# kamperh/segmentalist

Measured on AMD Instinct MI355X. Metric: Gibbs sweeps/sec (10k utts, D=100, K=1000) at 1/2/4/8 MI355X, higher is better.
Workload: dtype fp16 one-product filter + fp16x2 second stage, float32 reference arithmetic for the results; 1 GPU; SegmentalKMeansWordseg batch-synchronous sweep (BASELINE.json configs[2]); utterances=10000, landmarks_per_utt=20, n_slices_max=6, embeddings=1050000, D=100, K=1000, parallelism=utterance shards x1, ONE all-gather of the packed block statistics per sweep, collective=none (single process), sweep_launch=plain launches, corpus=one device holds all rows, device_memory_allocated_bytes_rank0=1237140992, components_after=815

## Files before the change

### include/segk.h

```cpp
#ifndef SEGK_H
#define SEGK_H

#include <stdint.h>

#ifdef __cplusplus
extern "C" {
#endif

#define SEGK_OK 0
#define SEGK_ERR_ARG (-1)
#define SEGK_ERR_HIP (-2)
#define SEGK_ERR_NO_DEVICE (-3)
#define SEGK_ERR_UNSUPPORTED (-4)

#define SEGK_F32 0
#define SEGK_F64 1

typedef struct segk_ctx segk_ctx;

int32_t segk_create(int32_t device_id, segk_ctx **out_ctx);
int32_t segk_destroy(segk_ctx *ctx);
const char *segk_last_error(void);
#define SEGK_ABI_VERSION 15
int32_t segk_abi_version(void);
// ... 103 lines not shown

int32_t segk_kmeans_update_utt(segk_ctx *ctx, const segk_corpus *c, segk_kmeans *m,
                               int32_t utt, const int32_t *old_tok, const int32_t *new_tok,
                               const int32_t *new_k, const int32_t *n_old, const int32_t *n_new,
                               int32_t *status, void *stream);

int32_t segk_kmeans_add_item(segk_ctx *ctx, const segk_corpus *c, segk_kmeans *m, int64_t i,
                             int32_t k, int32_t *status, void *stream);
int32_t segk_kmeans_del_item(segk_ctx *ctx, const segk_corpus *c, segk_kmeans *m, int64_t i,
                             int32_t *status, void *stream);
int32_t segk_kmeans_clean_components(segk_ctx *ctx, const segk_corpus *c, segk_kmeans *m,
                                     int32_t *status, void *stream);

int32_t segk_kmeans_del_component(segk_ctx *ctx, const segk_corpus *c, segk_kmeans *m, int32_t k,
                                  int32_t *status, void *stream);

int32_t segk_kmeans_sequential_sweep(segk_ctx *ctx, const segk_corpus *c, segk_kmeans *m,
                                     const int32_t *order, int32_t n_order, int32_t n_slices_min,
                                     int32_t n_slices_max, double wip, const segk_cand *cand,
                                     uint64_t *keys_scratch, uint8_t *boundaries, int32_t *old_tok,
                                     int32_t *new_tok, int32_t *new_k, int32_t *n_old, int32_t *n_new,
                                     int32_t *n_flag, double *out_total, int32_t *status, void *stream);

int64_t segk_kmeans_batch_record_words(int32_t K_max, int32_t D, int32_t n_blocks_local, int32_t flag_cap,
                                       int32_t flag_row_bytes);
int32_t segk_kmeans_batch_scratch_words(int32_t K_max, int64_t n_slots, int32_t n_blocks_local, int64_t *sorted_words,
                                        int64_t *koff_words);
int32_t segk_kmeans_batch_partials(segk_ctx *ctx, const segk_corpus *c, const segk_kmeans *m,
                                   const int32_t *blk_lo, int32_t n_blocks_local,
                                   const int32_t *new_tok, const int32_t *new_k, const int32_t *n_flag,
                                   const double *out_total, int32_t *sorted_scratch,
                                   int32_t *koff_scratch, double *record, int32_t flag_cap, int32_t flag_rows,
                                   double *out_scalars, void *stream);
int32_t segk_kmeans_batch_finalize(segk_ctx *ctx, const segk_corpus *c, segk_kmeans *m,
                                   int32_t utt_lo, int32_t utt_hi, const double *records,
                                   int32_t n_blocks_total, int32_t n_blocks_per_rank,
                                   int64_t rank_stride, int32_t flag_cap, int32_t flag_rows, int32_t my_rank,
                                   int32_t *new_k, int32_t *remap_scratch, double *out_scalars,
                                   int32_t *status, void *stream);
int32_t segk_kmeans_batch_record(segk_ctx *ctx, const segk_corpus *c, const segk_kmeans *m, int32_t utt_lo,
                                 int32_t utt_hi, const int32_t *new_tok, const int32_t *new_k,
                                 const int32_t *status, double *out_scalars, void *stream);
int32_t segk_kmeans_assignments_from_tokens(segk_ctx *ctx, const segk_corpus *c, segk_kmeans *m,
                                            int32_t utt_lo, int32_t utt_hi, const int32_t *new_tok,
                                            const int32_t *new_k, const int32_t *n_new,
                                            void *stream);

int64_t segk_kmeans_refit_scratch_words(int64_t n_slots);
int32_t segk_kmeans_refit_collect(segk_ctx *ctx, const segk_corpus *c, int32_t utt_lo, int32_t utt_hi,
                                  const int32_t *new_tok, const int32_t *new_k, int32_t *chunk_scratch,
                                  int32_t *ids, int32_t *slots, int64_t n_list, int32_t *count_out,
                                  int32_t *status, void *stream);
int32_t segk_kmeans_refit_apply(segk_ctx *ctx, const segk_corpus *c, const segk_kmeans *m,
                                const segk_cand *cand, int32_t utt_lo, int32_t utt_hi,
                                const int32_t *new_tok, int32_t *new_k, int32_t *n_flag, int32_t *moved,
                                int32_t *status, void *stream);
int32_t segk_kmeans_hint_relabel(segk_ctx *ctx, const segk_corpus *c, const segk_kmeans *m,
                                 const segk_cand *cand, const int32_t *table, void *stream);
int32_t segk_kmeans_refit_record(segk_ctx *ctx, const segk_corpus *c, const segk_kmeans *m, int32_t utt_lo,
                                 int32_t utt_hi, const int32_t *new_tok, const int32_t *new_k,
                                 const int32_t *status, const int32_t *moved, double *out_scalars,
                                 void *stream);

int64_t segk_kmeans_fit_scratch_words(int64_t n_emb, int64_t n_items_max, int32_t K_max);
int32_t segk_kmeans_fit_step(segk_ctx *ctx, const segk_corpus *c, segk_kmeans *m, const segk_cand *cand,
                             int32_t consider_unassigned, int64_t n_items_max, int32_t *scratch, double *record,
// ... 193 lines not shown
```

### segmentalist_amd/_abi.py

```python
import ctypes as C
import os
import subprocess

_HERE = os.path.dirname(os.path.abspath(__file__))
LIB_PATH = os.environ.get("SEGK_LIB_PATH") or os.path.join(_HERE, "libsegk.so")

SEGK_F32, SEGK_F64 = 0, 1
SEGK_ERR_UNSUPPORTED = -4
ABI_VERSION = 15


class SegkError(RuntimeError):
    pass


class Corpus(C.Structure):
    _fields_ = [
        ("X", C.c_void_p), ("X32", C.c_void_p), ("x_dtype", C.c_int32), ("D", C.c_int32),
        ("n_emb", C.c_int64), ("ldx", C.c_int64), ("ld32", C.c_int64), ("xnorm", C.c_void_p),
        ("vec_ids", C.c_void_p), ("durations", C.c_void_p), ("lengths", C.c_void_p),
        ("n_utt", C.c_int32), ("N_max", C.c_int32), ("Xb3", C.c_void_p), ("sp_pieces", C.c_int32), ("band_W", C.c_int32),
        ("band_ids", C.c_void_p), ("band_dur", C.c_void_p),
    ]

# ... 43 lines not shown
    "segk_create": (_i32, [_i32, C.POINTER(_P)]),
    "segk_destroy": (_i32, [_P]),
    "segk_last_error": (C.c_char_p, []),
    "segk_abi_version": (_i32, []),
    "segk_corpus_prepare": (_i32, [_P, _CP, _P, _P, _P]),
    "segk_kmeans_tiles_floats": (_i64, [_i32, _i32]),
    "segk_kmeans_prepare": (_i32, [_P, _CP, _KP, _P]),
    "segk_kmeans_mark_duplicates": (_i32, [_P, _CP, _KP, _P, _P]),
    "segk_kmeans_init_stats": (_i32, [_P, _CP, _KP, _P]),
    "segk_kmeans_score": (_i32, [_P, _CP, _KP, _P, _i64, _i64, _DP, _P, _P]),
    "segk_kmeans_score_hinted": (_i32, [_P, _CP, _KP, _P, _i64, _i64, _DP, _P, _P, _P]),
    "segk_kmeans_clear_queue": (_i32, [_P, _DP, _P]),
    "segk_kmeans_filter": (_i32, [_P, _CP, _KP, _P, _i64, _i64, _DP, _P]),
    "segk_kmeans_resolve": (_i32, [_P, _CP, _KP, _P, _i64, _i64, _DP, _P, _P]),
    "segk_kmeans_stage_counts": (_i32, [_P, _DP, C.POINTER(_i32), _P]),
    "segk_kmeans_hint_feedback": (_i32, [_P, C.POINTER(C.c_uint32), C.POINTER(C.c_uint32), C.POINTER(_i32)]),
    "segk_kmeans_delta_stats": (_i32, [_P, C.POINTER(_i32)]),
    "segk_kmeans_exact_max": (_i32, [_P, _CP, _KP, _P, _i64, _DP, _P, _P, _P]),
    "segk_kmeans_neg_sqrd_norm": (_i32, [_P, _CP, _KP, _i64, _P, _P]),
    "segk_kmeans_segment": (_i32, [_P, _CP, _KP, _P, _i32, _i32, _i32, _i32, _f64, _DP, _P, _P, _P, _P, _P, _P,
                                   _P, _P, _P, _P]),
    "segk_dp_tri": (_i32, [_P, _i32, _P, _P, _P, _i32, _i32, _i32, _f64, _f64, _P, _i64, _P, _i64, _P, _P, _P,
                           _P, _i64, _P]),
    "segk_kmeans_update_utt": (_i32, [_P, _CP, _KP, _i32, _P, _P, _P, _P, _P, _P, _P]),
    "segk_kmeans_sequential_sweep": (_i32, [_P, _CP, _KP, _P, _i32, _i32, _i32, _f64, _DP, _P, _P, _P, _P, _P, _P, _P, _P, _P,
                                            _P, _P]),
    "segk_kmeans_add_item": (_i32, [_P, _CP, _KP, _i64, _i32, _P, _P]),
    "segk_kmeans_del_item": (_i32, [_P, _CP, _KP, _i64, _P, _P]),
    "segk_kmeans_clean_components": (_i32, [_P, _CP, _KP, _P, _P]),
    "segk_kmeans_del_component": (_i32, [_P, _CP, _KP, _i32, _P, _P]),
    "segk_kmeans_batch_record_words": (_i64, [_i32, _i32, _i32, _i32, _i32]),
    "segk_kmeans_batch_scratch_words": (_i32, [_i32, _i64, _i32, C.POINTER(_i64), C.POINTER(_i64)]),
    "segk_kmeans_batch_partials": (_i32, [_P, _CP, _KP, _P, _i32, _P, _P, _P, _P, _P, _P, _P, _i32, _i32, _P, _P]),
    "segk_kmeans_batch_finalize": (_i32, [_P, _CP, _KP, _i32, _i32, _P, _i32, _i32, _i64, _i32, _i32, _i32, _P, _P, _P, _P,
                                          _P]),
    "segk_kmeans_batch_record": (_i32, [_P, _CP, _KP, _i32, _i32, _P, _P, _P, _P, _P]),
    "segk_kmeans_assignments_from_tokens": (_i32, [_P, _CP, _KP, _i32, _i32, _P, _P, _P, _P]),
    "segk_kmeans_refit_scratch_words": (_i64, [_i64]),
    "segk_kmeans_refit_collect": (_i32, [_P, _CP, _i32, _i32, _P, _P, _P, _P, _P, _i64, _P, _P, _P]),
    "segk_kmeans_refit_apply": (_i32, [_P, _CP, _KP, _DP, _i32, _i32, _P, _P, _P, _P, _P, _P]),
    "segk_kmeans_hint_relabel": (_i32, [_P, _CP, _KP, _DP, _P, _P]),
    "segk_kmeans_refit_record": (_i32, [_P, _CP, _KP, _i32, _i32, _P, _P, _P, _P, _P, _P]),
    "segk_kmeans_fit_scratch_words": (_i64, [_i64, _i64, _i32]),
    "segk_kmeans_fit_step": (_i32, [_P, _CP, _KP, _DP, _i32, _i64, _P, _P, _P, _P]),
    "segk_kmeans_sum_neg_sqrd_norm": (_i32, [_P, _CP, _KP, _P, _P]),
    "segk_fbgmm_record_metrics": (_i32, [_P, _CP, _FP, _i32, _f64, _P, _P]),
    "segk_fbgmm_init_stats": (_i32, [_P, _CP, _FP, _P]),
    "segk_fbgmm_update": (_i32, [_P, _CP, _FP, _i32, _i32, _i64, _i32, _P, _P]),
    "segk_fbgmm_score": (_i32, [_P, _CP, _FP, _P, _i64, _i64, _P, _P]),
    "segk_fbgmm_pred_vector": (_i32, [_P, _CP, _FP, _i64, _P, _P]),
    "segk_unigram_segment": (_i32, [_P, _CP, _i32, _i32, _i32, _i32, _f64, _f64, _f64, _f64, _P, _P, _P, _i64, _P,
                                    _P, _P, _P, _P, _P]),
    "segk_fbgmm_assign": (_i32, [_P, _CP, _FP, _i32, _i32, _i32, _f64, _P, _P, _P, _P, _i64, _P, _P]),
    "segk_fbgmm_gibbs_items": (_i32, [_P, _CP, _FP, _P, _i64, _i32, _f64, _P, _P, _i64, _P, _P]),
    "segk_fbgmm_sequential_sweep": (_i32, [_P, _CP, _FP, _P, _i32, _P, _i32, _i32, _i32, _i32, _f64, _f64, _f64, _f64, _f64,
                                           _P, _P, _P, _i64, _P, _P, _P, _P, _P, _P]),
    "segk_fbb_collect": (_i32, [_P, _CP, _P, _P, _P, _P]),
    "segk_fbb_partials": (_i32, [_P, _CP, _FP, _BP, _i32, _i32, _i32, _P, _P, _P]),
    "segk_fbb_prepare": (_i32, [_P, _CP, _FP, _BP, _i32, _P]),
    "segk_fbb_score": (_i32, [_P, _CP, _FP, _BP, _i32, _i32, _i32, _P, _P, _P]),
    "segk_fbb_score_diag32": (_i32, [_P, _CP, _FP, _BP, _i32, _i32, _i32, _P, _P, _P]),
    "segk_calibrate_vlog": (_i32, [_P, C.POINTER(_f64), _P]),
    "segk_fbb_make_y": (_i32, [_P, _CP, _BP, _P]),
    "segk_fbb_prior_rows": (_i32, [_P, _CP, _FP, _P, _P]),
    "segk_fbb_score_f32": (_i32, [_P, _CP, _FP, _BP, _P, _i64, _P, _P]),
    "segk_fbb_segment": (_i32, [_P, _CP, _FP, _BP, _i32, _i32, _i32, _P, _u64, _i32, _i32, _f64, _f64, _f64, _P, _P,
# ... 103 lines not shown
```

### segmentalist_amd/csrc/segk_stats.hip

```cpp
#include "segk_kmeans_dev.h"


template <typename XT>
__device__ void dev_del_component(const segk_corpus &c, segk_kmeans &m, int k, int *shK, int32_t *relog = nullptr)
{
    const int tid = threadIdx.x, nt = blockDim.x;
    const int D = c.D;
    const int K = *shK;
    XT *means = (XT *)m.means;
    const XT *rnd = (const XT *)m.random_means;
    if (k != K) {
        const double cntK = (double)m.counts[K];
        for (int d = tid; d < D; d += nt) {
            double v = m.mean_numerators[(int64_t)K * D + d];
            m.mean_numerators[(int64_t)k * D + d] = v;
            means[(int64_t)k * D + d] = (XT)(v / cntK);
        }
        if (relog) {
            if (tid == 0) {
                const int n = relog[0];
                relog[1 + 2 * n] = K;
                relog[2 + 2 * n] = k;
                relog[0] = n + 1;
            }
// ... 523 lines not shown
    double s = 0.0;
    for (int uc = u0; uc < u1; uc += 2048) {
        const int nu = u1 - uc < 2048 ? u1 - uc : 2048;
        __syncthreads();
        for (int i = tid; i < nu; i += SORT_THREADS) stage[i] = out_total[uc + i];
        __syncthreads();
        if (tid == 0) {
            int i = 0;
            for (; i + 16 <= nu; i += 16) {
                double v[16];
#pragma unroll
                for (int q = 0; q < 16; q++) v[q] = stage[i + q];
#pragma unroll
                for (int q = 0; q < 16; q++) s += v[q];
            }
            for (; i < nu; i++) s += stage[i];
        }
    }
    if (tid == 0) part_tot[b] = s;
    SEGK_TSTAMP(1, 4);
}

#define SORT_CL 512
static inline __host__ __device__ int segk_sort_rsh(int K_max) { return K_max <= 2048 ? 5 : 7; }
static inline __host__ __device__ int segk_sort_nsh(int K_max)
{
    const int need = (K_max + (1 << segk_sort_rsh(K_max)) - 1) >> segk_sort_rsh(K_max);
    int nsh = 0;
    while ((1 << nsh) < need) nsh++;
    return nsh;
}
static inline __host__ __device__ int segk_sort_ranges(int K_max) { return 1 << segk_sort_nsh(K_max); }

__global__ __launch_bounds__(SORT_THREADS) void k_batch_sort_sum(
    segk_corpus c, segk_kmeans m, const int32_t *blk_lo, int n_blocks, const int32_t *new_tok, const int32_t *new_k,
    const double *out_total, int32_t *sorted, int32_t *koff2, double *part_tot, int32_t *flags, int cap, double *out_scalars, int NR,
    int rsh, int nsh, double *part_sum, int64_t *part_cnt, int fuse_sum)
{
    extern __shared__ __attribute__((aligned(16))) unsigned char sort_lds[];
    __shared__ int32_t wcount[16], wscan[2];
    const int tid = threadIdx.x, lane = tid & 63, wv = tid >> 6;
    const int Kb = *m.K;
    const int K_max = m.K_max;
    const int RS = 1 << rsh, kmask = RS - 1;
    const int b = blockIdx.x / (NR + 2), r = blockIdx.x % (NR + 2);
    const int u0 = blk_lo[b], u1 = blk_lo[b + 1];
    SEGK_TSTAMP(1, 0);
    if (r == NR + 1) {
        if (b == 0 && tid == 0) {
            *(double *)m.mnorm_max = 0.0;
            out_scalars[3] = (double)Kb;
        }
        double *stage = reinterpret_cast<double *>(sort_lds);
        double s = 0.0;
        for (int uc = u0; uc < u1; uc += 2048) {
            const int nu = u1 - uc < 2048 ? u1 - uc : 2048;
            __syncthreads();
            for (int i = tid; i < nu; i += SORT_THREADS) stage[i] = out_total[uc + i];
            __syncthreads();
            if (tid == 0) {
                int i = 0;
                for (; i + 16 <= nu; i += 16) {
                    double v[16];
#pragma unroll
                    for (int q = 0; q < 16; q++) v[q] = stage[i + q];
#pragma unroll
                    for (int q = 0; q < 16; q++) s += v[q];
                }
                for (; i < nu; i++) s += stage[i];
            }
        }
        if (tid == 0) part_tot[b] = s;
        SEGK_TSTAMP(1, 4);
        return;
    }
    const bool flg = r == NR;
    const int64_t p0 = (int64_t)u0 * c.N_max;
    const int S = (u1 - u0) * c.N_max;
    const int per = ((S + 15) / 16 + 63) & ~63;
    const bool preload = per <= 2048;
    int32_t *cntw = reinterpret_cast<int32_t *>(sort_lds);
    int32_t *base = cntw + 16 * RS;
    int32_t *cnts = base + RS;
    uint32_t *cl = reinterpret_cast<uint32_t *>(cnts + RS) + (size_t)wv * SORT_CL;
    const int32_t *keys = new_k + (S > 0 ? p0 : 0);
    const int s0 = wv * per < S ? wv * per : S, s1 = s0 + per < S ? s0 + per : S;
    auto in_range = [&](int k) -> bool { return flg ? k >= Kb : (k >= 0 && k < Kb && (k & (NR - 1)) == r); };
    for (int i = tid; i < 16 * RS; i += SORT_THREADS) cntw[i] = 0;
    int n_mine = 0;
    if (preload) {
        constexpr int NC = 2048 / 64;
        int v[NC];
#pragma unroll
        for (int q = 0; q < NC; q++) {
            const int sidx = s0 + q * 64 + lane;
            v[q] = keys[sidx < s1 ? sidx : (S > 0 ? S - 1 : 0)];
        }
        __syncthreads();
#pragma unroll
        for (int q = 0; q < NC; q++) {
            if (s0 + q * 64 >= s1) break;
            const int sidx = s0 + q * 64 + lane;
            const int k = sidx < s1 ? v[q] : -1;
            const bool in = sidx < s1 && in_range(k);
            const unsigned long long bal = __ballot(in);
            if (in) {
                const int at = n_mine + __popcll(bal & ((1ull << lane) - 1ull));
                if (at < SORT_CL) cl[at] = ((unsigned int)sidx << rsh) | (unsigned int)((k >> nsh) & kmask);
                if (!flg) atomicAdd(&cntw[wv * RS + ((k >> nsh) & kmask)], 1);
            }
            n_mine += __popcll(bal);
        }
    } else {
        __syncthreads();
        for (int sb = s0; sb < s1; sb += 64) {
            const int sidx = sb + lane;
            const int k = sidx < s1 ? keys[sidx] : -1;
            const bool in = sidx < s1 && in_range(k);
            if (in && !flg) atomicAdd(&cntw[wv * RS + ((k >> nsh) & kmask)], 1);
            n_mine += __popcll(__ballot(in));
        }
    }
    if (lane == 0) wcount[wv] = n_mine;
    const bool compact = !__syncthreads_or(!preload || n_mine > SORT_CL);
    SEGK_TSTAMP(1, 2);
    if (flg) {
        int32_t *fl = flags + (int64_t)b * 2 * segk_flag_words(cap);
        int off = 0, tot = 0;
        for (int w = 0; w < 16; w++) {
            if (w < wv) off += wcount[w];
            tot += wcount[w];
        }
        if (tid == 0) { fl[0] = tot; fl[1] = 0; }
        if (compact) {
            for (int i = lane; i < n_mine; i += 64) {
                const int sidx = (int)(cl[i] >> rsh);
                if (off + i < cap) {
                    fl[2 + 3 * (off + i) + 0] = (int32_t)(p0 + sidx);
                    fl[2 + 3 * (off + i) + 1] = keys[sidx];
                    fl[2 + 3 * (off + i) + 2] = new_tok[p0 + sidx];
                }
            }
        } else {
            int done = 0;
            for (int sb = s0; sb < s1 && done < n_mine; sb += 64) {
                const int sidx = sb + lane;
                const int k = sidx < s1 ? keys[sidx] : -1;
                const bool in = sidx < s1 && k >= Kb;
                const unsigned long long bal = __ballot(in);
                const int at = off + done + __popcll(bal & ((1ull << lane) - 1ull));
                if (in && at < cap) {
                    fl[2 + 3 * at + 0] = (int32_t)(p0 + sidx);
                    fl[2 + 3 * at + 1] = k;
                    fl[2 + 3 * at + 2] = new_tok[p0 + sidx];
                }
                done += __popcll(bal);
            }
        }
        SEGK_TSTAMP_MAX(1, 4);
        return;
    }
    int run = 0, incl = 0;
    if (tid < RS) {
        int t[16];
#pragma unroll
        for (int w = 0; w < 16; w++) t[w] = cntw[w * RS + tid];
#pragma unroll
        for (int w = 0; w < 16; w++) {
            cntw[w * RS + tid] = run;
            run += t[w];
        }
        incl = run;
        for (int o = 1; o < 64; o <<= 1) {
            const int t2 = __shfl_up(incl, o);
            if (lane >= o) incl += t2;
        }
        if (lane == 63) wscan[wv] = incl;
    }
    __syncthreads();
    if (tid < RS) {
        const int ex = (wv == 1 ? wscan[0] : 0) + incl - run;
        base[tid] = ex;
        cnts[tid] = run;
        const int k = (tid << nsh) + r;
        if (k < K_max) {
            koff2[((int64_t)b * K_max + k) * 2 + 0] = ex;
            koff2[((int64_t)b * K_max + k) * 2 + 1] = run;
        }
    }
    __syncthreads();
    SEGK_TSTAMP(1, 3);
    int32_t *region = sorted + p0 * NR + (int64_t)r * S;
    int32_t *mine = cntw + wv * RS;
    if (compact) {
        for (int ib = 0; ib < n_mine; ib += 64) {
            const int i = ib + lane;
            const bool ok = i < n_mine;
            const unsigned int e = ok ? cl[i] : 0u;
            const int kk = (int)(e & (unsigned int)kmask);
            const int row = new_tok[p0 + (ok ? (int)(e >> rsh) : 0)];
            const unsigned long long same = dev_match_key(kk, ok, rsh);
            if (ok) {
                const int rank = __popcll(same & ((1ull << lane) - 1ull));
                const int before = mine[kk];
                region[base[kk] + before + rank] = row;
                if (rank == __popcll(same) - 1) mine[kk] = before + rank + 1;
            }
        }
    } else {
        for (int sb = s0; sb < s1; sb += 64) {
            const int sidx = sb + lane;
            const int k = sidx < s1 ? keys[sidx] : -1;
            const bool ok = sidx < s1 && in_range(k);
            if (__ballot(ok) == 0ull) continue;
            const int kk = (k >> nsh) & kmask;
            const unsigned long long same = dev_match_key(kk, ok, rsh);
            if (ok) {
                const int rank = __popcll(same & ((1ull << lane) - 1ull));
                const int before = mine[kk];
                region[base[kk] + before + rank] = new_tok[p0 + sidx];
                if (rank == __popcll(same) - 1) mine[kk] = before + rank + 1;
            }
        }
    }
    SEGK_TSTAMP_MAX(1, 4);
    if (!fuse_sum) return;
    __syncthreads();
    {
        const int T = base[RS - 1] + cnts[RS - 1];
        auto owner = [&](int kk) -> int {
            const int o = T > 0 ? (int)(((long long)base[kk] * 16) / T) : 0;
            return o < 15 ? o : 15;
        };
        const unsigned long long m0 = __ballot(lane < RS && owner(lane < RS ? lane : 0) == wv),
                                 m1 = __ballot(64 + lane < RS && owner(64 + lane < RS ? 64 + lane : 0) == wv);
        if ((m0 | m1) == 0ull) return;
        const int ka = m0 ? __ffsll((long long)m0) - 1 : 64 + __ffsll((long long)m1) - 1;
        const int kb = m1 ? 128 - __clzll((long long)m1) : 64 - __clzll((long long)m0);
        const int D = c.D;
        const float *Xf = (const float *)c.X;
        const int dl = 2 * lane < D ? 2 * lane : 0;
        const int t_lo = base[ka], t_hi = base[kb - 1] + cnts[kb - 1];
        double a0 = 0.0, a1 = 0.0;
        int kk = ka, rem = cnts[ka];
        auto flush = [&]() {
            for (;;) {
                const int k = (kk << nsh) + r;
                if (k < K_max) {
                    if (2 * lane < D) *reinterpret_cast<double2 *>(part_sum + ((int64_t)b * K_max + k) * D + 2 * lane) = make_double2(a0, a1);
                    if (lane == 0) part_cnt[(int64_t)b * K_max + k] = cnts[kk];
                }
                a0 = 0.0;
                a1 = 0.0;
                kk++;
                if (kk >= kb) { rem = 0x7fffffff; return; }
                rem = cnts[kk];
                if (rem > 0) return;
            }
        };
        if (rem == 0) flush();
        for (int c0 = t_lo; c0 < t_hi; c0 += 64) {
            const int nb = t_hi - c0 < 64 ? t_hi - c0 : 64;
            const int mine_row = region[c0 + (lane < nb ? lane : 0)];
            for (int q0 = 0; q0 < nb; q0 += 32) {
                float2 xv[32];
#pragma unroll
                for (int q = 0; q < 32; q++) {
                    const int e = __shfl(mine_row, q0 + q < nb ? q0 + q : 0);
                    xv[q] = *reinterpret_cast<const float2 *>(Xf + (int64_t)e * c.ldx + dl);
                }
#pragma unroll
                for (int q = 0; q < 32; q++) {
                    if (q0 + q < nb) {
                        a0 += (double)xv[q].x;
                        a1 += (double)xv[q].y;
                        if (--rem == 0) flush();
                    }
                }
            }
        }
        SEGK_TSTAMP_MAX(1, 5);
    }
}

#define PART_WAVES 4
template <typename XT>
__global__ __launch_bounds__(64 * PART_WAVES) void k_batch_partials(segk_corpus c, segk_kmeans m, const int32_t *blk_lo, int n_blocks,
                                                                   const int32_t *sorted, const int32_t *koff2,
                                                                   double *part_sum, int64_t *part_cnt, int NR)
{
    const int groups = (m.K_max + PART_WAVES - 1) / PART_WAVES;
    const int b = blockIdx.x / groups, kg = blockIdx.x % groups;
    const int wv = threadIdx.x >> 6, lane = threadIdx.x & 63;
    const int k = kg * PART_WAVES + wv;
    SEGK_TSTAMP(2, 0);
    if (k >= m.K_max) return;
    const int D = c.D;
    const XT *X = (const XT *)c.X;
    const int2 on = *reinterpret_cast<const int2 *>(koff2 + ((int64_t)b * m.K_max + k) * 2);
    const int nm = on.y;
#ifdef SEGK_STAMP
    if (segk_tstamp_buf && lane == 0 && (unsigned long long)nm > *SEGK_TSTAMP_AT(2, 2)) *SEGK_TSTAMP_AT(2, 2) = (unsigned long long)nm;
#endif
    const int64_t p0 = (int64_t)blk_lo[b] * c.N_max;
    const int S = (blk_lo[b + 1] - blk_lo[b]) * c.N_max;
    const int32_t *list = sorted + p0 * NR + (int64_t)(k & (NR - 1)) * S + on.x;
    double *out = part_sum + ((int64_t)b * m.K_max + k) * D;
    if (lane == 0) part_cnt[(int64_t)b * m.K_max + k] = nm;
    constexpr int MAXR = 2;
// ... 841 lines not shown
    segk_delta_pending_drop(ctx);
    rc = launch_update(c, m, 3, 0, 0, 0, nullptr, nullptr, nullptr, nullptr, nullptr, status, (hipStream_t)stream);
    if (rc) return rc;
    return segk_kmeans_prepare(ctx, c, m, stream);
}

int32_t segk_kmeans_del_component(segk_ctx *ctx, const segk_corpus *c, segk_kmeans *m, int32_t k,
                                  int32_t *status, void *stream)
{
    int rc = check_corpus(c);
    if (rc) return rc;
    segk_delta_pending_drop(ctx);
    SEGK_REQUIRE(k >= 0 && k < m->K_max, "k out of range");
    rc = launch_update(c, m, 4, 0, 0, k, nullptr, nullptr, nullptr, nullptr, nullptr, status, (hipStream_t)stream);
    if (rc) return rc;
    return segk_kmeans_prepare(ctx, c, m, stream);
}

int32_t segk_kmeans_batch_scratch_words(int32_t K_max, int64_t n_slots, int32_t n_blocks_local, int64_t *sorted_words,
                                        int64_t *koff_words)
{
    SEGK_REQUIRE(K_max >= 1 && n_slots >= 0 && n_blocks_local >= 0 && sorted_words && koff_words, "batch_scratch_words operands");
    *sorted_words = (n_slots > 0 ? n_slots : 1) * segk_sort_ranges(K_max);
    *koff_words = (int64_t)(n_blocks_local > 0 ? n_blocks_local : 1) * K_max * 2;
    return SEGK_OK;
}

int64_t segk_kmeans_batch_record_words(int32_t K_max, int32_t D, int32_t n_blocks_local, int32_t flag_cap, int32_t flag_row_bytes)
{
    const int64_t rw = flag_row_bytes > 0 ? ((int64_t)flag_cap * flag_row_bytes + 7) / 8 : 0;
    return (int64_t)n_blocks_local * ((int64_t)K_max * D + 1 + K_max + segk_flag_words(flag_cap) + rw);
}

int32_t segk_kmeans_batch_partials(segk_ctx *ctx, const segk_corpus *c, const segk_kmeans *m,
                                   const int32_t *blk_lo, int32_t n_blocks_local,
                                   const int32_t *new_tok, const int32_t *new_k, const int32_t *n_flag,
                                   const double *out_total, int32_t *sorted_scratch, int32_t *koff_scratch,
                                   double *record, int32_t flag_cap, int32_t flag_rows, double *out_scalars, void *stream)
{
    (void)ctx;
    int rc = check_corpus(c);
    if (rc) return rc;
    if (n_blocks_local <= 0) return SEGK_OK;
    SEGK_REQUIRE(blk_lo && new_tok && new_k && n_flag && out_total && record && out_scalars && sorted_scratch && koff_scratch,
                 "batch_partials operands");
    SEGK_REQUIRE(flag_cap >= 1, "flag_cap");
    SEGK_REQUIRE(m->K_max <= 8192, "batch mode supports K_max <= 8192");
    const int64_t nbl = n_blocks_local, KD = (int64_t)m->K_max * c->D;
    double *part_sum = record;
    double *part_tot = record + nbl * KD;
    int64_t *part_cnt = reinterpret_cast<int64_t *>(record + nbl * KD + nbl);
    int32_t *flags = reinterpret_cast<int32_t *>(record + nbl * KD + nbl + nbl * m->K_max);
    hipStream_t st = (hipStream_t)stream;
    (void)n_flag;
    segk_tstamp_bind();
    const int NR = segk_sort_ranges(m->K_max), rsh = segk_sort_rsh(m->K_max), nsh = segk_sort_nsh(m->K_max);
    const bool fuse = c->x_dtype == SEGK_F32 && c->D <= 128 && (c->D & 1) == 0 && (c->ldx & 1) == 0;
    {
        size_t lds = (size_t)(16 + 2) * (1 << rsh) * 4 + (size_t)16 * SORT_CL * 4;
        if (lds < 2048 * sizeof(double)) lds = 2048 * sizeof(double);
        hipLaunchKernelGGL(k_batch_sort_sum, dim3((unsigned)(nbl * (NR + 2))), dim3(SORT_THREADS), lds, st, *c, *m, blk_lo,
                           n_blocks_local, new_tok, new_k, out_total, sorted_scratch, koff_scratch, part_tot, flags, flag_cap,
                           out_scalars, NR, rsh, nsh, part_sum, part_cnt, fuse ? 1 : 0);
        SEGK_LAUNCH_CHECK();
    }
    if (flag_rows) {
        const int elem = c->x_dtype == SEGK_F32 ? 4 : 8;
        const int64_t rw = segk_flag_row_words(flag_cap, c->D, elem);
        double *rows = record + nbl * KD + nbl + nbl * m->K_max + nbl * segk_flag_words(flag_cap);
        DISPATCH_XT(c, hipLaunchKernelGGL(k_batch_flag_rows<XT>, dim3((unsigned)nbl), dim3(256), 0, st, *c, flags, flag_cap, (XT *)rows, rw););
        SEGK_LAUNCH_CHECK();
    }
    if (fuse) return SEGK_OK;
    const int64_t grid = nbl * ((m->K_max + PART_WAVES - 1) / PART_WAVES);
    DISPATCH_XT(c, hipLaunchKernelGGL(k_batch_partials<XT>, dim3((unsigned)grid), dim3(64 * PART_WAVES), 0, st, *c, *m, blk_lo,
                                       n_blocks_local, sorted_scratch, koff_scratch, part_sum, part_cnt, NR););
    SEGK_LAUNCH_CHECK();
    return SEGK_OK;
}

int32_t segk_kmeans_batch_finalize(segk_ctx *ctx, const segk_corpus *c, segk_kmeans *m, int32_t utt_lo,
                                   int32_t utt_hi, const double *records, int32_t n_blocks_total,
                                   int32_t n_blocks_per_rank, int64_t rank_stride, int32_t flag_cap, int32_t flag_rows,
                                   int32_t my_rank, int32_t *new_k, int32_t *remap_scratch, double *out_scalars, int32_t *status,
                                   void *stream)
{
    int rc = check_corpus(c);
    if (rc) return rc;
    SEGK_REQUIRE(n_blocks_total >= 1 && n_blocks_total <= 64, "1 <= n_blocks_total <= 64");
    SEGK_REQUIRE(n_blocks_per_rank >= 1 && n_blocks_total % n_blocks_per_rank == 0, "blocks per rank");
    SEGK_REQUIRE(m->K_max <= 8192, "batch mode supports K_max <= 8192");
    SEGK_REQUIRE(records && new_k && remap_scratch && out_scalars && status && m->tiles && m->mnorm_max, "batch_finalize operands");
    SEGK_REQUIRE(0 <= utt_lo && utt_lo <= utt_hi && utt_hi <= c->n_utt, "utterance range");
    hipStream_t st = (hipStream_t)stream;
    segk_delta_pending_drop(ctx);
    unsigned long long *row_hash = nullptr;
// ... 131 lines not shown
```

### segmentalist_amd/device.py

```python
import ctypes as C
import os

import numpy as np

from . import _abi
from ._abi import SEGK_F32, SEGK_F64, SegkError, check, ptr
from .comm import SingleComm, get_comm

AM32_TILE_MIN = 15000


def _torch():
    import torch
    return torch


def _dev():
    torch = _torch()
    if not torch.cuda.is_available():
        raise SegkError("segmentalist_amd needs an MI355X: no ROCm device is visible and there is no "
                        "CPU fallback for the hot path")
    return torch.device("cuda", torch.cuda.current_device())


# ... 439 lines not shown
                lo_b, hi_b = int(self.bounds[b]), int(self.bounds[b + 1])
                lo = lo_b + (j * (hi_b - lo_b)) // n_batches
                hi = lo_b + ((j + 1) * (hi_b - lo_b)) // n_batches
                utts.append(np.arange(lo, hi, dtype=np.int32))
                rows.append(np.arange(int(self._row_start[lo]), int(self._row_start[hi]), dtype=np.int32))
            u, r = np.concatenate(utts), np.concatenate(rows)
            contiguous = self.nbl == 1 or (len(u) and u[-1] - u[0] + 1 == len(u))
            steps.append((u, r, bool(contiguous)))
        return steps


class KMeansBatchSweeper(object):

    def __init__(self, dk, part, flag_cap=4096, group=None):
        torch = _torch()
        dev = _dev()
        self.dk, self.part, self.cap, self.comm = dk, part, int(flag_cap), get_comm(group)
        assert self.comm.world == part.world and self.comm.rank == part.rank
        c = dk.corpus
        W = part.world
        self.flag_rows = 1 if dk.shard is not None else 0
        self.rank_stride = int(dk._L.segk_kmeans_batch_record_words(
            dk.K_max, c.D, part.nbl, self.cap, c.D * (4 if c.x_dtype == SEGK_F32 else 8) if self.flag_rows else 0))
        self.pack_all = torch.zeros((W, self.rank_stride), dtype=torch.float64, device=dev)
        self.pack = self.pack_all[part.rank]
        self.blk_lo = to_dev(part.local_bounds, np.int32)
        ws, wk = C.c_int64(), C.c_int64()
        n_loc = (part.utt_hi - part.utt_lo) * c.N_max
        check(dk._L.segk_kmeans_batch_scratch_words(dk.K_max, n_loc, part.nbl, C.byref(ws), C.byref(wk)))
        self.sorted = torch.zeros(ws.value, dtype=torch.int32, device=dev)
        nr = ws.value // max(n_loc, 1)
        self._sorted_ptr = C.c_void_p(self.sorted.data_ptr() - 4 * part.utt_lo * c.N_max * nr)
        self.koff = torch.zeros(wk.value, dtype=torch.int32, device=dev)
        import os
        self.use_graph = os.environ.get("SEGK_SWEEP_GRAPH", "0") == "1"
        self._graph, self._graph_args, self._side, self._warm = None, None, None, 0
        self._sweeps_done = 0
        _l, _s, _p = C.c_uint32(0), C.c_uint32(0), C.c_int32(0)
        check(dk._L.segk_kmeans_hint_feedback(dk._ctx, C.byref(_l), C.byref(_s), C.byref(_p)))
        self._fb_seen = _l.value
        self._mb = None
        self._hints_current = False
        self._refits_done = 0
        self._refit = None
        self._n_tok = None
        dk.batch_comm = self.comm

    HINT_MISS_PERMILLE = 450

    def _use_hints(self):
        if self._sweeps_done < 2:
            return False
        launched, seen, permille = C.c_uint32(0), C.c_uint32(0), C.c_int32(0)
        check(self.dk._L.segk_kmeans_hint_feedback(self.dk._ctx, C.byref(launched), C.byref(seen), C.byref(permille)))
        if seen.value > self._fb_seen:
            self._fb_seen = seen.value
            if permille.value > self.HINT_MISS_PERMILLE:
                return False
        return True

    def _minibatch_tables(self, n_batches):
        if self._mb is None or self._mb[0] != n_batches:
            steps = []
            for u, r, contiguous in self.part.minibatch(n_batches):
                r = r - self.dk.row_base
                if contiguous:
# ... 1 lines not shown
                else:
                    steps.append((0, len(u), 0, len(r), to_dev(u, np.int32), to_dev(r, np.int32)))
            self._mb = (n_batches, steps)
        return self._mb[1]

    def _tokens_from_state(self, boundaries):
        torch = _torch()
        dk, c = self.dk, self.dk.corpus
        check(dk._L.segk_fbb_collect(dk._ctx, dk._cp(), ptr(boundaries), ptr(dk.new_tok), ptr(dk.n_new), _abi.stream()))
        live = torch.arange(c.N_max, device=dk.n_new.device, dtype=torch.int32)[None, :] < dk.n_new[:, None]
        lab = dk.assignments[dk.new_tok.clamp(min=0).long()]
        dk.new_k.copy_(torch.where(live, lab, torch.full_like(lab, -1)))
        dk.n_flag.zero_()

    def sweep_minibatch(self, boundaries, n_slices_min, n_slices_max, wip, n_batches):
        dk, pt = self.dk, self.part
        L, ctx, cp, mp, st = dk._L, dk._ctx, dk._cp(), C.byref(dk.m), _abi.stream()
        if dk.assign_stale is None:
            dk.ensure_boundaries()
            self._tokens_from_state(boundaries)
        hints = self._use_hints()
        self._n_tok = None
        for (utt0, n_utts, row0, n_rows, utts, rows) in self._minibatch_tables(n_batches):
            hint = {} if not hints else {"hint_identity": True} if self._hints_current else {"hint_remap": dk.remap}
            self._hints_current = False
            if rows is None:
                dk.score_rows(row0=row0, n=n_rows, **hint)
                dk.segment(boundaries, n_slices_min, n_slices_max, wip, utt0=utt0, n_utts=n_utts)
            else:
                dk.score_rows(ids=rows, **hint)
                check(L.segk_kmeans_segment(ctx, cp, mp, ptr(utts), 0, n_utts, int(n_slices_min), int(n_slices_max), float(wip),
                                            C.byref(dk.cand), ptr(boundaries), ptr(dk.old_tok), ptr(dk.new_tok), ptr(dk.new_k),
                                            ptr(dk.n_old), ptr(dk.n_new), ptr(dk.n_flag), ptr(dk.out_total), ptr(dk.status), st))
            check(L.segk_kmeans_batch_partials(ctx, cp, mp, ptr(self.blk_lo), pt.nbl, ptr(dk.new_tok), ptr(dk.new_k),
                                               ptr(dk.n_flag), ptr(dk.out_total), self._sorted_ptr, ptr(self.koff),
                                               ptr(self.pack), self.cap, self.flag_rows, ptr(dk.out_scalars), st))
            if pt.world > 1:
                self.comm.all_gather_rows(self.pack_all, self.pack)
            self._enqueue_back()
        self._sweeps_done += 1
        dk.assign_stale = (pt.utt_lo, pt.utt_hi, pt.world)
        dk.bounds_stale = (boundaries, pt) if pt.world > 1 else None

    def _enqueue_front(self, boundaries, n_slices_min, n_slices_max, wip):
        dk, pt = self.dk, self.part
        L, ctx, cp, mp, st = dk._L, dk._ctx, dk._cp(), C.byref(dk.m), _abi.stream()
        hint = {} if not self._use_hints() else {"hint_identity": True} if self._hints_current else {"hint_remap": dk.remap}
        dk.score_rows(row0=pt.row_lo - dk.row_base, n=pt.row_hi - pt.row_lo, **hint)
        dk.segment(boundaries, n_slices_min, n_slices_max, wip, utt0=pt.utt_lo, n_utts=pt.utt_hi - pt.utt_lo)
        check(L.segk_kmeans_batch_partials(ctx, cp, mp, ptr(self.blk_lo), pt.nbl, ptr(dk.new_tok), ptr(dk.new_k),
                                           ptr(dk.n_flag), ptr(dk.out_total), self._sorted_ptr, ptr(self.koff),
                                           ptr(self.pack), self.cap, self.flag_rows, ptr(dk.out_scalars), st))

    def _enqueue_back(self):
        dk, pt = self.dk, self.part
        L, ctx, cp, mp, st = dk._L, dk._ctx, dk._cp(), C.byref(dk.m), _abi.stream()
        check(L.segk_kmeans_batch_finalize(ctx, cp, mp, pt.utt_lo, pt.utt_hi, ptr(self.pack_all), pt.n_blocks, pt.nbl,
                                           self.rank_stride, self.cap, self.flag_rows, pt.rank, ptr(dk.new_k), ptr(dk.remap),
                                           ptr(dk.out_scalars), ptr(dk.status), st))

    def sweep(self, boundaries, n_slices_min, n_slices_max, wip):
        dk, pt = self.dk, self.part
        if self.use_graph:
            self._sweep_graph(boundaries, n_slices_min, n_slices_max, wip)
        else:
            self._enqueue_front(boundaries, n_slices_min, n_slices_max, wip)
            if pt.world > 1:
                self.comm.all_gather_rows(self.pack_all, self.pack)
            self._enqueue_back()
        dk.assign_stale = (pt.utt_lo, pt.utt_hi, pt.world)
        dk.bounds_stale = (boundaries, pt) if pt.world > 1 else None
        self._sweeps_done += 1
        self._hints_current = False
        self._n_tok = None

    def note_token_count(self, n):
        self._n_tok = int(n)

    def _relabel_hints(self):
        dk = self.dk
        check(dk._L.segk_kmeans_hint_relabel(dk._ctx, dk._cp(), C.byref(dk.m), C.byref(dk.cand), ptr(dk.remap), _abi.stream()))

    def refit(self, boundaries):
        torch = _torch()
        dk, pt, c = self.dk, self.part, self.dk.corpus
        L, ctx, cp, mp, st = dk._L, dk._ctx, dk._cp(), C.byref(dk.m), _abi.stream()
        if dk.assign_stale is None:
            dk.ensure_boundaries()
            self._tokens_from_state(boundaries)
            self._n_tok = None
        if self.use_graph:
            self._drop_graph()
            self._warm = 0
        n_slots = (pt.utt_hi - pt.utt_lo) * c.N_max
        if self._refit is None:
            bound = min(int(c.lengths_np[pt.utt_lo:pt.utt_hi].sum()), n_slots, c.n_emb)
            dev = dk.new_k.device
            self._refit = (torch.zeros(max(bound, 1), dtype=torch.int32, device=dev),
                           torch.zeros(int(L.segk_kmeans_refit_scratch_words(n_slots)), dtype=torch.int32, device=dev),
                           torch.zeros(1, dtype=torch.int32, device=dev), bound)
        ids, chunks, count, bound = self._refit
        n_list = bound if self._n_tok is None else min(self._n_tok, bound)
        hints = self._use_hints()
        if not self._hints_current and self._sweeps_done + self._refits_done > 0:
            self._relabel_hints()
        check(L.segk_kmeans_refit_collect(ctx, cp, pt.utt_lo, pt.utt_hi, ptr(dk.new_tok), ptr(dk.new_k), ptr(chunks), ptr(ids),
                                          None, n_list, ptr(count), ptr(dk.status), st))
        dk.score_rows(ids=ids[:n_list], hint_identity=hints)
        check(L.segk_kmeans_refit_apply(ctx, cp, mp, C.byref(dk.cand), pt.utt_lo, pt.utt_hi, ptr(dk.new_tok), ptr(dk.new_k),
                                        ptr(dk.n_flag), ptr(dk.refit_moved), ptr(dk.status), st))
        check(L.segk_kmeans_batch_partials(ctx, cp, mp, ptr(self.blk_lo), pt.nbl, ptr(dk.new_tok), ptr(dk.new_k),
                                           ptr(dk.n_flag), ptr(dk.out_total), self._sorted_ptr, ptr(self.koff),
                                           ptr(self.pack), self.cap, self.flag_rows, ptr(dk.out_scalars), st))
        if pt.world > 1:
            self.comm.all_gather_rows(self.pack_all, self.pack)
        self._enqueue_back()
        self._relabel_hints()
        self._hints_current = True
        self._refits_done += 1
        dk.assign_stale = (pt.utt_lo, pt.utt_hi, pt.world)

    def _capture(self, fn):
        dk = self.dk
        st = _abi.stream()
        check(dk._L.segk_graph_begin(dk._ctx, st))
        try:
            fn()
        finally:
            ex = C.c_void_p()
            rc = dk._L.segk_graph_end(dk._ctx, st, C.byref(ex))
        check(rc)
        return ex

    def _sweep_graph(self, boundaries, n_slices_min, n_slices_max, wip):
        torch = _torch()
        dk, pt = self.dk, self.part
        args = (boundaries.data_ptr(), int(n_slices_min), int(n_slices_max), float(wip))
        cur = torch.cuda.current_stream()
        if self._side is None:
            self._side = torch.cuda.Stream()
        self._side.wait_stream(cur)
        with torch.cuda.stream(self._side):
            if self._warm < 1 or (self._graph is not None and self._graph_args != args):
                self._drop_graph()
            if self._warm < 1:
                self._enqueue_front(boundaries, n_slices_min, n_slices_max, wip)
# ... 763 lines not shown
```

Before: 7377 sweeps/s.

## Skip re-summing cluster embeddings whose sorted membership is unchanged since last sweep

The fused sort-and-sum kernel now keeps a per-(block, range) record holding a header of shapes and buffer pointers. It loads the previous sorted member list and the per-cluster offsets, then compares each cluster's newly scattered rows against the previous ones. Clusters whose member rows are identical keep their earlier partial sums, so their embedding gather and accumulation is skipped. This aims to cut the large gather-and-accumulate cost once assignments settle. In exchange it adds LDS use, extra compare work in the scatter, and a dependency on the sum buffers persisting unchanged between calls. It can be turned off with an environment variable.

```diff
diff --git a/include/segk.h b/include/segk.h
--- a/include/segk.h
+++ b/include/segk.h
@@ -159,6 +159,13 @@
                                    const double *out_total, int32_t *sorted_scratch,
                                    int32_t *koff_scratch, double *record, int32_t flag_cap, int32_t flag_rows,
                                    double *out_scalars, void *stream);
+int64_t segk_kmeans_batch_keep_words(int32_t K_max, int32_t n_blocks_local);
+int32_t segk_kmeans_batch_partials_keep(segk_ctx *ctx, const segk_corpus *c, const segk_kmeans *m,
+                                        const int32_t *blk_lo, int32_t n_blocks_local,
+                                        const int32_t *new_tok, const int32_t *new_k, const int32_t *n_flag,
+                                        const double *out_total, int32_t *sorted_scratch,
+                                        int32_t *koff_scratch, double *record, int32_t flag_cap, int32_t flag_rows,
+                                        double *out_scalars, void *stream, int32_t *keep, int64_t keep_words);
 int32_t segk_kmeans_batch_finalize(segk_ctx *ctx, const segk_corpus *c, segk_kmeans *m,
                                    int32_t utt_lo, int32_t utt_hi, const double *records,
                                    int32_t n_blocks_total, int32_t n_blocks_per_rank,
diff --git a/segmentalist_amd/_abi.py b/segmentalist_amd/_abi.py
--- a/segmentalist_amd/_abi.py
+++ b/segmentalist_amd/_abi.py
@@ -99,6 +99,8 @@
     "segk_kmeans_batch_record_words": (_i64, [_i32, _i32, _i32, _i32, _i32]),
     "segk_kmeans_batch_scratch_words": (_i32, [_i32, _i64, _i32, C.POINTER(_i64), C.POINTER(_i64)]),
     "segk_kmeans_batch_partials": (_i32, [_P, _CP, _KP, _P, _i32, _P, _P, _P, _P, _P, _P, _P, _i32, _i32, _P, _P]),
+    "segk_kmeans_batch_partials_keep": (_i32, [_P, _CP, _KP, _P, _i32, _P, _P, _P, _P, _P, _P, _P, _i32, _i32, _P, _P, _P, _i64]),
+    "segk_kmeans_batch_keep_words": (_i64, [_i32, _i32]),
     "segk_kmeans_batch_finalize": (_i32, [_P, _CP, _KP, _i32, _i32, _P, _i32, _i32, _i64, _i32, _i32, _i32, _P, _P, _P, _P,
                                           _P]),
     "segk_kmeans_batch_record": (_i32, [_P, _CP, _KP, _i32, _i32, _P, _P, _P, _P, _P]),
diff --git a/segmentalist_amd/csrc/segk_stats.hip b/segmentalist_amd/csrc/segk_stats.hip
--- a/segmentalist_amd/csrc/segk_stats.hip
+++ b/segmentalist_amd/csrc/segk_stats.hip
@@ -579,10 +579,45 @@
 }
 static inline __host__ __device__ int segk_sort_ranges(int K_max) { return 1 << segk_sort_nsh(K_max); }
 
+#define KEEP_MAGIC 0x6b656570
+#define KEEP_HDR 20
+#define KEEP_REC 32
+#ifndef KEEP_CAP
+#define KEEP_CAP 4096
+#endif
+static_assert(KEEP_CAP % SORT_THREADS == 0 && KEEP_CAP / SORT_THREADS <= 4, "KEEP_CAP");
+static __device__ __forceinline__ int32_t keep_hdr_word(int i, const segk_corpus &c, int K_max, int u0, int u1, int NR, const void *sorted,
+                                                         const void *koff2, const void *part_sum, int live)
+{
+    const unsigned long long ax = (unsigned long long)c.X, as = (unsigned long long)sorted, ak = (unsigned long long)koff2,
+                             ap = (unsigned long long)part_sum;
+    switch (i) {
+    case 0: return live ? KEEP_MAGIC : 0;
+    case 1: return u0;
+    case 2: return u1;
+    case 3: return NR;
+    case 4: return c.D;
+    case 5: return (int32_t)c.ldx;
+    case 6: return (int32_t)c.n_emb;
+    case 7: return c.N_max;
+    case 8: return K_max;
+    case 9: return c.x_dtype;
+    case 10: return (int32_t)ax;
+    case 11: return (int32_t)(ax >> 32);
+    case 12: return (int32_t)as;
+    case 13: return (int32_t)(as >> 32);
+    case 14: return (int32_t)ak;
+    case 15: return (int32_t)(ak >> 32);
+    case 16: return (int32_t)ap;
+    case 17: return (int32_t)(ap >> 32);
+    default: return 0;
+    }
+}
+
 __global__ __launch_bounds__(SORT_THREADS) void k_batch_sort_sum(
     segk_corpus c, segk_kmeans m, const int32_t *blk_lo, int n_blocks, const int32_t *new_tok, const int32_t *new_k,
     const double *out_total, int32_t *sorted, int32_t *koff2, double *part_tot, int32_t *flags, int cap, double *out_scalars, int NR,
-    int rsh, int nsh, double *part_sum, int64_t *part_cnt, int fuse_sum)
+    int rsh, int nsh, double *part_sum, int64_t *part_cnt, int fuse_sum, int32_t *keep, int keep_mode)
 {
     extern __shared__ __attribute__((aligned(16))) unsigned char sort_lds[];
     __shared__ int32_t wcount[16], wscan[2];
@@ -634,6 +669,25 @@
     const int s0 = wv * per < S ? wv * per : S, s1 = s0 + per < S ? s0 + per : S;
     auto in_range = [&](int k) -> bool { return flg ? k >= Kb : (k >= 0 && k < Kb && (k & (NR - 1)) == r); };
     for (int i = tid; i < 16 * RS; i += SORT_THREADS) cntw[i] = 0;
+    int32_t *region = sorted + p0 * NR + (int64_t)r * S;
+    int32_t *prev = reinterpret_cast<int32_t *>(cnts + RS) + 16 * SORT_CL;
+    int32_t *keepf = prev + KEEP_CAP;
+    int32_t *kshift = keepf + RS;
+    int32_t *krec = keep && !flg ? keep + ((int64_t)b * NR + r) * KEEP_REC : nullptr;
+    const bool kp = krec && keep_mode == 1 && fuse_sum;
+    const int prevn = S < KEEP_CAP ? S : KEEP_CAP;
+    int hexp = 0, hgot = 0, pv[KEEP_CAP / SORT_THREADS];
+    int2 kold = make_int2(0, 0);
+    if (krec && tid < KEEP_HDR) hexp = keep_hdr_word(tid, c, K_max, u0, u1, NR, sorted, koff2, part_sum, kp ? 1 : 0);
+    if (kp) {
+        if (tid < KEEP_HDR) hgot = krec[tid];
+        if (tid < RS && (tid << nsh) + r < K_max) kold = *reinterpret_cast<const int2 *>(koff2 + ((int64_t)b * K_max + (tid << nsh) + r) * 2);
+#pragma unroll
+        for (int j = 0; j < KEEP_CAP / SORT_THREADS; j++) {
+            const int i = j * SORT_THREADS + tid;
+            pv[j] = prevn > 0 ? region[i < prevn ? i : 0] : 0;
+        }
+    }
     int n_mine = 0;
     if (preload) {
         constexpr int NC = 2048 / 64;
@@ -669,7 +723,12 @@
         }
     }
     if (lane == 0) wcount[wv] = n_mine;
+    if (kp) {
+#pragma unroll
+        for (int j = 0; j < KEEP_CAP / SORT_THREADS; j++) prev[j * SORT_THREADS + tid] = pv[j];
+    }
     const bool compact = !__syncthreads_or(!preload || n_mine > SORT_CL);
+    const bool keep_ok = !__syncthreads_or(!kp || (tid < KEEP_HDR && hgot != hexp));
     SEGK_TSTAMP(1, 2);
     if (flg) {
         int32_t *fl = flags + (int64_t)b * 2 * segk_flag_words(cap);
@@ -734,10 +793,12 @@
             koff2[((int64_t)b * K_max + k) * 2 + 0] = ex;
             koff2[((int64_t)b * K_max + k) * 2 + 1] = run;
         }
+        const bool cand = keep_ok && run > 0 && kold.y == run && kold.x >= 0 && kold.x <= prevn - run;
+        keepf[tid] = cand ? 1 : 0;
+        kshift[tid] = cand ? kold.x - ex : 0;
     }
     __syncthreads();
     SEGK_TSTAMP(1, 3);
-    int32_t *region = sorted + p0 * NR + (int64_t)r * S;
     int32_t *mine = cntw + wv * RS;
     if (compact) {
         for (int ib = 0; ib < n_mine; ib += 64) {
@@ -750,7 +811,9 @@
             if (ok) {
                 const int rank = __popcll(same & ((1ull << lane) - 1ull));
                 const int before = mine[kk];
-                region[base[kk] + before + rank] = row;
+                const int pos = base[kk] + before + rank;
+                region[pos] = row;
+                if (keep_ok && keepf[kk] && prev[pos + kshift[kk]] != row) keepf[kk] = 0;
                 if (rank == __popcll(same) - 1) mine[kk] = before + rank + 1;
             }
         }
@@ -765,16 +828,37 @@
             if (ok) {
                 const int rank = __popcll(same & ((1ull << lane) - 1ull));
                 const int before = mine[kk];
-                region[base[kk] + before + rank] = new_tok[p0 + sidx];
+                const int pos = base[kk] + before + rank, row = new_tok[p0 + sidx];
+                region[pos] = row;
+                if (keep_ok && keepf[kk] && prev[pos + kshift[kk]] != row) keepf[kk] = 0;
                 if (rank == __popcll(same) - 1) mine[kk] = before + rank + 1;
             }
         }
     }
     SEGK_TSTAMP_MAX(1, 4);
-    if (!fuse_sum) return;
+    if (krec && tid < KEEP_HDR) krec[tid] = hexp;
+    if (!fuse_sum) {
+        if (krec && tid == 0) krec[KEEP_HDR] = krec[KEEP_HDR + 1] = 0;
+        return;
+    }
     __syncthreads();
     {
         const int T = base[RS - 1] + cnts[RS - 1];
+        unsigned long long kq0 = 0ull, kq1 = 0ull;
+        if (keep_ok) {
+            kq0 = __ballot(lane < RS && keepf[lane < RS ? lane : 0] != 0);
+            kq1 = __ballot(64 + lane < RS && keepf[64 + lane < RS ? 64 + lane : 0] != 0);
+        }
+        auto kept = [&](int kk) -> bool { return ((kk < 64 ? kq0 >> kk : kq1 >> (kk - 64)) & 1ull) != 0ull; };
+        if (krec && wv == 0) {
+            const int live = __popcll(__ballot(lane < RS && cnts[lane < RS ? lane : 0] > 0)) +
+                             __popcll(__ballot(64 + lane < RS && cnts[64 + lane < RS ? 64 + lane : 0] > 0));
+            const int nk = __popcll(kq0) + __popcll(kq1);
+            if (lane == 0) {
+                krec[KEEP_HDR] = nk;
+                krec[KEEP_HDR + 1] = live - nk;
+            }
+        }
         auto owner = [&](int kk) -> int {
             const int o = T > 0 ? (int)(((long long)base[kk] * 16) / T) : 0;
             return o < 15 ? o : 15;
@@ -787,9 +871,8 @@
         const int D = c.D;
         const float *Xf = (const float *)c.X;
         const int dl = 2 * lane < D ? 2 * lane : 0;
-        const int t_lo = base[ka], t_hi = base[kb - 1] + cnts[kb - 1];
         double a0 = 0.0, a1 = 0.0;
-        int kk = ka, rem = cnts[ka];
+        int kk = ka, rem = 0, cb = kb;
         auto flush = [&]() {
             for (;;) {
                 const int k = (kk << nsh) + r;
@@ -800,28 +883,39 @@
                 a0 = 0.0;
                 a1 = 0.0;
                 kk++;
-                if (kk >= kb) { rem = 0x7fffffff; return; }
+                if (kk >= cb) { rem = 0x7fffffff; return; }
                 rem = cnts[kk];
                 if (rem > 0) return;
             }
         };
-        if (rem == 0) flush();
-        for (int c0 = t_lo; c0 < t_hi; c0 += 64) {
-            const int nb = t_hi - c0 < 64 ? t_hi - c0 : 64;
-            const int mine_row = region[c0 + (lane < nb ? lane : 0)];
-            for (int q0 = 0; q0 < nb; q0 += 32) {
-                float2 xv[32];
-#pragma unroll
-                for (int q = 0; q < 32; q++) {
-                    const int e = __shfl(mine_row, q0 + q < nb ? q0 + q : 0);
-                    xv[q] = *reinterpret_cast<const float2 *>(Xf + (int64_t)e * c.ldx + dl);
-                }
-#pragma unroll
-                for (int q = 0; q < 32; q++) {
-                    if (q0 + q < nb) {
-                        a0 += (double)xv[q].x;
-                        a1 += (double)xv[q].y;
-                        if (--rem == 0) flush();
+        for (int ca = ka; ca < kb; ca = cb) {
+            cb = ca + 1;
+            if (kept(ca)) continue;
+            while (cb < kb && !kept(cb)) cb++;
+            const int t_lo = base[ca], t_hi = base[cb - 1] + cnts[cb - 1];
+            a0 = 0.0;
+            a1 = 0.0;
+            kk = ca;
+            rem = cnts[ca];
+            if (rem == 0) flush();
+            for (int c0 = t_lo; c0 < t_hi; c0 += 64) {
+                const int nb = t_hi - c0 < 64 ? t_hi - c0 : 64;
+                const int mine_row = kp ? __hip_atomic_load(region + c0 + (lane < nb ? lane : 0), __ATOMIC_RELAXED, __HIP_MEMORY_SCOPE_AGENT)
+                                        : region[c0 + (lane < nb ? lane : 0)];
+                for (int q0 = 0; q0 < nb; q0 += 32) {
+                    float2 xv[32];
+#pragma unroll
+                    for (int q = 0; q < 32; q++) {
+                        const int e = __shfl(mine_row, q0 + q < nb ? q0 + q : 0);
+                        xv[q] = *reinterpret_cast<const float2 *>(Xf + (int64_t)e * c.ldx + dl);
+                    }
+#pragma unroll
+                    for (int q = 0; q < 32; q++) {
+                        if (q0 + q < nb) {
+                            a0 += (double)xv[q].x;
+                            a1 += (double)xv[q].y;
+                            if (--rem == 0) flush();
+                        }
                     }
                 }
             }
@@ -1729,11 +1823,44 @@
     return (int64_t)n_blocks_local * ((int64_t)K_max * D + 1 + K_max + segk_flag_words(flag_cap) + rw);
 }
 
+int64_t segk_kmeans_batch_keep_words(int32_t K_max, int32_t n_blocks_local)
+{
+    if (K_max < 1) return 0;
+    return (int64_t)(n_blocks_local > 0 ? n_blocks_local : 1) * segk_sort_ranges(K_max) * KEEP_REC;
+}
+
+static int32_t batch_partials(segk_ctx *ctx, const segk_corpus *c, const segk_kmeans *m, const int32_t *blk_lo, int32_t n_blocks_local,
+                              const int32_t *new_tok, const int32_t *new_k, const int32_t *n_flag, const double *out_total,
+                              int32_t *sorted_scratch, int32_t *koff_scratch, double *record, int32_t flag_cap, int32_t flag_rows,
+                              double *out_scalars, void *stream, int32_t *keep, int keep_mode);
+
 int32_t segk_kmeans_batch_partials(segk_ctx *ctx, const segk_corpus *c, const segk_kmeans *m,
                                    const int32_t *blk_lo, int32_t n_blocks_local,
                                    const int32_t *new_tok, const int32_t *new_k, const int32_t *n_flag,
                                    const double *out_total, int32_t *sorted_scratch, int32_t *koff_scratch,
                                    double *record, int32_t flag_cap, int32_t flag_rows, double *out_scalars, void *stream)
+{
+    return batch_partials(ctx, c, m, blk_lo, n_blocks_local, new_tok, new_k, n_flag, out_total, sorted_scratch, koff_scratch, record,
+                          flag_cap, flag_rows, out_scalars, stream, nullptr, 0);
+}
+
+int32_t segk_kmeans_batch_partials_keep(segk_ctx *ctx, const segk_corpus *c, const segk_kmeans *m,
+                                        const int32_t *blk_lo, int32_t n_blocks_local,
+                                        const int32_t *new_tok, const int32_t *new_k, const int32_t *n_flag,
+                                        const double *out_total, int32_t *sorted_scratch, int32_t *koff_scratch,
+                                        double *record, int32_t flag_cap, int32_t flag_rows, double *out_scalars, void *stream,
+                                        int32_t *keep, int64_t keep_words)
+{
+    SEGK_REQUIRE(!keep || keep_words >= segk_kmeans_batch_keep_words(m->K_max, n_blocks_local), "keep_words");
+    const char *e = getenv("SEGK_BATCH_KEEP");
+    return batch_partials(ctx, c, m, blk_lo, n_blocks_local, new_tok, new_k, n_flag, out_total, sorted_scratch, koff_scratch, record,
+                          flag_cap, flag_rows, out_scalars, stream, keep, keep ? (e && e[0] == '0' && !e[1] ? 2 : 1) : 0);
+}
+
+static int32_t batch_partials(segk_ctx *ctx, const segk_corpus *c, const segk_kmeans *m, const int32_t *blk_lo, int32_t n_blocks_local,
+                              const int32_t *new_tok, const int32_t *new_k, const int32_t *n_flag, const double *out_total,
+                              int32_t *sorted_scratch, int32_t *koff_scratch, double *record, int32_t flag_cap, int32_t flag_rows,
+                              double *out_scalars, void *stream, int32_t *keep, int keep_mode)
 {
     (void)ctx;
     int rc = check_corpus(c);
@@ -1754,11 +1881,11 @@
     const int NR = segk_sort_ranges(m->K_max), rsh = segk_sort_rsh(m->K_max), nsh = segk_sort_nsh(m->K_max);
     const bool fuse = c->x_dtype == SEGK_F32 && c->D <= 128 && (c->D & 1) == 0 && (c->ldx & 1) == 0;
     {
-        size_t lds = (size_t)(16 + 2) * (1 << rsh) * 4 + (size_t)16 * SORT_CL * 4;
+        size_t lds = (size_t)(16 + 2) * (1 << rsh) * 4 + (size_t)16 * SORT_CL * 4 + (size_t)KEEP_CAP * 4 + (size_t)2 * (1 << rsh) * 4;
         if (lds < 2048 * sizeof(double)) lds = 2048 * sizeof(double);
         hipLaunchKernelGGL(k_batch_sort_sum, dim3((unsigned)(nbl * (NR + 2))), dim3(SORT_THREADS), lds, st, *c, *m, blk_lo,
                            n_blocks_local, new_tok, new_k, out_total, sorted_scratch, koff_scratch, part_tot, flags, flag_cap,
-                           out_scalars, NR, rsh, nsh, part_sum, part_cnt, fuse ? 1 : 0);
+                           out_scalars, NR, rsh, nsh, part_sum, part_cnt, fuse ? 1 : 0, keep, keep_mode);
         SEGK_LAUNCH_CHECK();
     }
     if (flag_rows) {
diff --git a/segmentalist_amd/device.py b/segmentalist_amd/device.py
--- a/segmentalist_amd/device.py
+++ b/segmentalist_amd/device.py
@@ -495,6 +495,7 @@
         nr = ws.value // max(n_loc, 1)
         self._sorted_ptr = C.c_void_p(self.sorted.data_ptr() - 4 * part.utt_lo * c.N_max * nr)
         self.koff = torch.zeros(wk.value, dtype=torch.int32, device=dev)
+        self.keep = torch.zeros(int(dk._L.segk_kmeans_batch_keep_words(dk.K_max, part.nbl)), dtype=torch.int32, device=dev)
         import os
         self.use_graph = os.environ.get("SEGK_SWEEP_GRAPH", "0") == "1"
         self._graph, self._graph_args, self._side, self._warm = None, None, None, 0
@@ -562,9 +563,10 @@
                 check(L.segk_kmeans_segment(ctx, cp, mp, ptr(utts), 0, n_utts, int(n_slices_min), int(n_slices_max), float(wip),
                                             C.byref(dk.cand), ptr(boundaries), ptr(dk.old_tok), ptr(dk.new_tok), ptr(dk.new_k),
                                             ptr(dk.n_old), ptr(dk.n_new), ptr(dk.n_flag), ptr(dk.out_total), ptr(dk.status), st))
-            check(L.segk_kmeans_batch_partials(ctx, cp, mp, ptr(self.blk_lo), pt.nbl, ptr(dk.new_tok), ptr(dk.new_k),
-                                               ptr(dk.n_flag), ptr(dk.out_total), self._sorted_ptr, ptr(self.koff),
-                                               ptr(self.pack), self.cap, self.flag_rows, ptr(dk.out_scalars), st))
+            check(L.segk_kmeans_batch_partials_keep(ctx, cp, mp, ptr(self.blk_lo), pt.nbl, ptr(dk.new_tok), ptr(dk.new_k),
+                                                    ptr(dk.n_flag), ptr(dk.out_total), self._sorted_ptr, ptr(self.koff),
+                                                    ptr(self.pack), self.cap, self.flag_rows, ptr(dk.out_scalars), st,
+                                                    ptr(self.keep), self.keep.numel()))
             if pt.world > 1:
                 self.comm.all_gather_rows(self.pack_all, self.pack)
             self._enqueue_back()
@@ -578,9 +580,10 @@
         hint = {} if not self._use_hints() else {"hint_identity": True} if self._hints_current else {"hint_remap": dk.remap}
         dk.score_rows(row0=pt.row_lo - dk.row_base, n=pt.row_hi - pt.row_lo, **hint)
         dk.segment(boundaries, n_slices_min, n_slices_max, wip, utt0=pt.utt_lo, n_utts=pt.utt_hi - pt.utt_lo)
-        check(L.segk_kmeans_batch_partials(ctx, cp, mp, ptr(self.blk_lo), pt.nbl, ptr(dk.new_tok), ptr(dk.new_k),
-                                           ptr(dk.n_flag), ptr(dk.out_total), self._sorted_ptr, ptr(self.koff),
-                                           ptr(self.pack), self.cap, self.flag_rows, ptr(dk.out_scalars), st))
+        check(L.segk_kmeans_batch_partials_keep(ctx, cp, mp, ptr(self.blk_lo), pt.nbl, ptr(dk.new_tok), ptr(dk.new_k),
+                                                ptr(dk.n_flag), ptr(dk.out_total), self._sorted_ptr, ptr(self.koff),
+                                                ptr(self.pack), self.cap, self.flag_rows, ptr(dk.out_scalars), st,
+                                                ptr(self.keep), self.keep.numel()))
 
     def _enqueue_back(self):
         dk, pt = self.dk, self.part
@@ -639,9 +642,10 @@
         dk.score_rows(ids=ids[:n_list], hint_identity=hints)
         check(L.segk_kmeans_refit_apply(ctx, cp, mp, C.byref(dk.cand), pt.utt_lo, pt.utt_hi, ptr(dk.new_tok), ptr(dk.new_k),
                                         ptr(dk.n_flag), ptr(dk.refit_moved), ptr(dk.status), st))
-        check(L.segk_kmeans_batch_partials(ctx, cp, mp, ptr(self.blk_lo), pt.nbl, ptr(dk.new_tok), ptr(dk.new_k),
-                                           ptr(dk.n_flag), ptr(dk.out_total), self._sorted_ptr, ptr(self.koff),
-                                           ptr(self.pack), self.cap, self.flag_rows, ptr(dk.out_scalars), st))
+        check(L.segk_kmeans_batch_partials_keep(ctx, cp, mp, ptr(self.blk_lo), pt.nbl, ptr(dk.new_tok), ptr(dk.new_k),
+                                                ptr(dk.n_flag), ptr(dk.out_total), self._sorted_ptr, ptr(self.koff),
+                                                ptr(self.pack), self.cap, self.flag_rows, ptr(dk.out_scalars), st,
+                                                ptr(self.keep), self.keep.numel()))
         if pt.world > 1:
             self.comm.all_gather_rows(self.pack_all, self.pack)
         self._enqueue_back()
```

Result: faster. 7595 sweeps/s, median of 6 (+3.0%).
